# mspaintenjoyer/DepthEstimation

Hardware: AMD Instinct MI355X
Metric: disparity Mpix/s at 1080p d_max=128; 1/2/4/8-GPU scaling + %HBM roofline (higher is better)
Workload: dtype u8

## Files before the change

### depthestimation_amd/csrc/dsx_bm.hip

```cpp
#include "dsx_internal.h"
#include "dsx_partition.h"
#include "dsx_subpix.h"

constexpr int kWpe = 3;
constexpr int kWpeSsd = 4;

#ifndef DSX_ROWSTEP_PAIRTAIL
#define DSX_ROWSTEP_PAIRTAIL 0
#endif
#ifndef DSX_ROWSTEP_DIVQ
#define DSX_ROWSTEP_DIVQ 1
#endif
constexpr bool kRowstepPairtail = DSX_ROWSTEP_PAIRTAIL;
constexpr bool kRowstepDivq = DSX_ROWSTEP_DIVQ;
#ifndef DSX_ROWSTEP_ATID
#define DSX_ROWSTEP_ATID 1
#endif
#ifndef DSX_ROWSTEP_KEY2
#define DSX_ROWSTEP_KEY2 1
#endif
#ifndef DSX_ROWSTEP_MERGE
#define DSX_ROWSTEP_MERGE 1
#endif
constexpr bool kRowstepMerge = DSX_ROWSTEP_MERGE;
constexpr bool kRowstepAtid = DSX_ROWSTEP_ATID;
constexpr bool kRowstepKey2 = DSX_ROWSTEP_KEY2;

#include <algorithm>
#include <cstdio>
#include <cstdlib>
#include <cstring>
#include <mutex>
#include <type_traits>
#include <utility>
#include <vector>

namespace dsx {

typedef unsigned short u16x2 __attribute__((ext_vector_type(2)));
typedef uint32_t u32x2 __attribute__((ext_vector_type(2)));
__device__ __forceinline__ u32x2 lds_read_b64(const uint8_t *p) {
    return *(const volatile __attribute__((address_space(3))) u32x2 *)p;
}

__device__ __forceinline__ u16x2 as2(uint32_t v) { return __builtin_bit_cast(u16x2, v); }
__device__ __forceinline__ uint32_t as1(u16x2 v) { return __builtin_bit_cast(uint32_t, v); }
__device__ __forceinline__ int clampi2(int v, int lo, int hi) { return v < lo ? lo : (v > hi ? hi : v); }
__device__ __forceinline__ uint32_t umin2(uint32_t a, uint32_t b) { return a < b ? a : b; }
__device__ __forceinline__ u16x2 add_sub2(u16x2 a, u16x2 p, u16x2 q) { return as2(as1(a) + as1(p) - as1(q)); }
__device__ __forceinline__ int mad_i24(int a, int b, int c) {
    int r;
    asm("v_mad_i32_i24 %0, %1, %2, %3" : "=v"(r) : "v"(a), "v"(b), "v"(c));
    return r;
}
__device__ __forceinline__ uint32_t sad_hi_u8(uint32_t a, uint32_t b, uint32_t c) {
    return __builtin_amdgcn_sad_hi_u8(a, b, c);
}
__device__ __forceinline__ uint32_t min_shr1(uint32_t src, uint32_t key) {
    asm("s_nop 1\n\tv_min_u32_dpp %0, %1, %0 wave_shr:1 row_mask:0xf bank_mask:0xf" : "+v"(key) : "v"(src));
    return key;
}
#pragma clang diagnostic push
#pragma clang diagnostic ignored "-Winline-asm"
template <int OFF0, int STRIDE>
__device__ __forceinline__ void lds_store8_addtid(uint32_t m0base, const uint32_t (&v)[8]) {
    static_assert(OFF0 >= 0 && OFF0 + 7 * STRIDE < 65536, "16-bit offset field");
    asm volatile("s_mov_b32 m0, %8\n\ts_nop 0\n\t"
                 "ds_write_addtid_b32 %0 offset:%9\n\t"
                 "ds_write_addtid_b32 %1 offset:%10\n\t"
                 "ds_write_addtid_b32 %2 offset:%11\n\t"
                 "ds_write_addtid_b32 %3 offset:%12\n\t"
                 "ds_write_addtid_b32 %4 offset:%13\n\t"
                 "ds_write_addtid_b32 %5 offset:%14\n\t"
                 "ds_write_addtid_b32 %6 offset:%15\n\t"
                 "ds_write_addtid_b32 %7 offset:%16"
                 :
                 : "v"(v[0]), "v"(v[1]), "v"(v[2]), "v"(v[3]), "v"(v[4]), "v"(v[5]), "v"(v[6]), "v"(v[7]), "s"(m0base),
                   "n"(OFF0), "n"(OFF0 + STRIDE), "n"(OFF0 + 2 * STRIDE), "n"(OFF0 + 3 * STRIDE), "n"(OFF0 + 4 * STRIDE),
                   "n"(OFF0 + 5 * STRIDE), "n"(OFF0 + 6 * STRIDE), "n"(OFF0 + 7 * STRIDE)
                 : "memory", "m0");
}
#pragma clang diagnostic pop
__device__ __forceinline__ void lds_drain() { asm volatile("s_waitcnt lgkmcnt(0)" ::: "memory"); }
__device__ __forceinline__ uint32_t lds_offset(const uint8_t *p) {
    return (uint32_t)(uintptr_t)(const __attribute__((address_space(3))) uint8_t *)p;
}
__host__ __device__ constexpr int rnd16(int v) { return (v + 15) & ~15; }
template <int R, bool SSD, int NW>
struct Geo {
    static constexpr int TX = 32;
    static constexpr int NC = TX + 2 * R;
    static constexpr int KD = SSD ? 1 : 2;
    static constexpr int LDW = 64 * KD;
    static constexpr int Dp = NW * LDW;
    static constexpr int NT = 64 * NW;
    static constexpr int TPP = NT / TX;
    static constexpr int DSL = Dp / TPP;
    static constexpr int CB = SSD ? 4 : 2;
    static constexpr int PITCH = Dp * CB + 16;
    static constexpr int NJ = NC + Dp;
    static constexpr int REFW = rnd16(NC + 4);
    static constexpr int SROW = rnd16(NJ * 4 + 16);
    static constexpr int MAXJ = (NJ + NT - 1) / NT;
    static constexpr int NB = DSL / 8;
    static constexpr int REFB = rnd16(4 * (NC + 8));
    static constexpr int SLOT = SROW + REFB;
    static constexpr int SMEM0 = 4 * SLOT + TX * PITCH;
    static constexpr int SMEM = SMEM0 > (2 * R + 1) * SLOT ? SMEM0 : (2 * R + 1) * SLOT;
    static constexpr int XRB = 128;
};

#ifdef DSX_STAMPS
#define DSX_STAMP(i)                                                                        \
    do {                                                                                    \
        __builtin_amdgcn_sched_barrier(0);                                                  \
        uint64_t t_;                                                                        \
        asm volatile("s_memtime %0\n\ts_waitcnt lgkmcnt(0)" : "=s"(t_)::"memory");          \
        __builtin_amdgcn_sched_barrier(0);                                                  \
        if ((i) > 0) ph[(i)-1] += t_ - t_prev;                                              \
        t_prev = t_;                                                                        \
    } while (0)
#else
#define DSX_STAMP(i) \
    do {             \
    } while (0)
#endif

__device__ __forceinline__ void lds_barrier() {
    __builtin_amdgcn_fence(__ATOMIC_RELEASE, "workgroup", "local");
    __builtin_amdgcn_s_barrier();
    __builtin_amdgcn_fence(__ATOMIC_ACQUIRE, "workgroup", "local");
}

template <int NW>
__device__ __forceinline__ void block_sync() {
    if constexpr (NW == 1) {
        __builtin_amdgcn_fence(__ATOMIC_ACQ_REL, "wavefront", "local");
    } else {
        lds_barrier();
    }
}

template <int TPP>
__device__ __forceinline__ uint32_t gmin(uint32_t v) {
    if constexpr (TPP > 1) v = umin2(v, (uint32_t)__builtin_amdgcn_update_dpp(0, (int)v, 0xB1, 0xF, 0xF, false));
    if constexpr (TPP > 2) v = umin2(v, (uint32_t)__builtin_amdgcn_update_dpp(0, (int)v, 0x4E, 0xF, 0xF, false));
    if constexpr (TPP > 4) v = umin2(v, (uint32_t)__builtin_amdgcn_ds_swizzle((int)v, 0x101F));
    if constexpr (TPP > 8) v = umin2(v, (uint32_t)__builtin_amdgcn_ds_swizzle((int)v, 0x201F));
    return v;
}


typedef const __attribute__((address_space(4))) uint32_t cu32;
typedef const __attribute__((address_space(1))) uint8_t gu8;
typedef const __attribute__((address_space(1))) uint32_t gu32;
typedef __attribute__((address_space(1))) uint8_t gw8;
typedef __attribute__((address_space(1))) int16_t g16;
typedef __attribute__((address_space(1))) float gf32;

template <bool RELOAD>
__device__ __forceinline__ Bm2Args kargs_row(const Bm2Args &a) {
    if constexpr (RELOAD) {
        typedef __attribute__((address_space(4))) const Bm2Args KArgs;
        KArgs *p = (KArgs *)__builtin_amdgcn_kernarg_segment_ptr();
        asm volatile("" : "+s"(p));
// ... 231 lines not shown
            } else {
                uint32_t v = 0;
#pragma unroll
                for (int q = 0; q < 4; ++q) v |= (uint32_t)srow[clampi2(PB - 4 * tj - q, 0, W - 1)] << (8 * (3 - q));
                w = v;
                e = srow[clampi2(PB - 4 * tj - 4, 0, W - 1)];
                v = 0;
#pragma unroll
                for (int q = 0; q < 4; ++q) v |= (uint32_t)rrow[clampi2(x0 - R + 4 * tr + q, 0, W - 1)] << (8 * q);
                rf = v;
            }
        };
#pragma unroll 1
        for (int g = 0; g < NGR; ++g) {
            uint32_t w[4], e[4], rf[4];
#pragma unroll
            for (int r = 0; r < 4; ++r) {
                if (4 * g + r <= 2 * R) {
                    ldb(yb - R + 4 * g + r, w[r], e[r], rf[r]);
                } else {
                    w[r] = 0;
                    e[r] = 0;
                    rf[r] = 0;
                }
            }
            uint32_t P[5];
#pragma unroll
            for (int q = 0; q < 4; ++q) {
                const uint32_t b = 3 - q;
                const uint32_t lo = __builtin_amdgcn_perm(w[1], w[0], 0x0C0C0000u | ((4u + b) << 8) | b);
                const uint32_t hi = __builtin_amdgcn_perm(w[3], w[2], 0x0C0C0000u | ((4u + b) << 8) | b);
                P[q] = __builtin_amdgcn_perm(hi, lo, 0x05040100u);
            }
            {
                const uint32_t lo = __builtin_amdgcn_perm(e[1], e[0], 0x0C0C0400u);
                const uint32_t hi = __builtin_amdgcn_perm(e[3], e[2], 0x0C0C0400u);
                P[4] = __builtin_amdgcn_perm(hi, lo, 0x05040100u);
            }
            if (tid < NJ4) {
                uint4 *tp = reinterpret_cast<uint4 *>(smem + g * TPG + 32 * tid);
                tp[0] = make_uint4(P[0], P[1], P[1], P[2]);
                tp[1] = make_uint4(P[2], P[3], P[3], P[4]);
            }
            if (tid < NC4) {
                uint32_t Rv[4];
#pragma unroll
                for (int k = 0; k < 4; ++k) {
                    const uint32_t lo = __builtin_amdgcn_perm(rf[1], rf[0], 0x0C0C0000u | ((4u + k) << 8) | (uint32_t)k);
                    const uint32_t hi = __builtin_amdgcn_perm(rf[3], rf[2], 0x0C0C0000u | ((4u + k) << 8) | (uint32_t)k);
                    Rv[k] = __builtin_amdgcn_perm(hi, lo, 0x05040100u);
                }
                *reinterpret_cast<uint4 *>(smem + NGR * TPG + g * RG + 16 * tid) = make_uint4(Rv[0], Rv[1], Rv[2], Rv[3]);
            }
        }
        block_sync<NW>();
        const uint8_t *tb = smem + d0 * 8;
        {
        uint32_t ae[NC], ao[NC];
#pragma unroll
        for (int c = 0; c < NC; ++c) ae[c] = ao[c] = 0;
#pragma unroll 1
        for (int g = 0; g < NGR; ++g) {
#pragma unroll
            for (int q = 0; q < NC4; ++q) {
                const int c0 = 4 * q;
                const uint4 rr = *reinterpret_cast<const uint4 *>(smem + NGR * TPG + g * RG + 4 * c0);
                const uint32_t rv[4] = {rr.x, rr.y, rr.z, rr.w};
#pragma unroll
                for (int c = 0; c < 4; ++c) {
                    if (c0 + c < NC) {
                        if constexpr (ABS) {
                            const uint32_t p0 = *reinterpret_cast<const uint32_t *>(tb + g * TPG + (NC - 1 - c0 - c) * 8);
                            ae[c0 + c] = __builtin_amdgcn_sad_u8(rv[c], p0, ae[c0 + c]);
                        } else {
                            const uint2 pr = *reinterpret_cast<const uint2 *>(tb + g * TPG + (NC - 1 - c0 - c) * 8);
                            ae[c0 + c] = __builtin_amdgcn_sad_u8(rv[c], pr.x, ae[c0 + c]);
                            ao[c0 + c] = __builtin_amdgcn_sad_u8(rv[c], pr.y, ao[c0 + c]);
                        }
                    }
                }
            }
        }
#pragma unroll
        for (int c = 0; c < NC; ++c) {
            if constexpr (ABS) cs[c] = ae[c];
            else cs[c] = as2(ae[c] | (ao[c] << 16));
        }
        }

    } else {
    block_sync<NW>();
    {
        constexpr int IG = 3;
#pragma unroll 1
        for (int i0 = 0; i0 <= 2 * R; i0 += IG) {
            uint32_t iw[IG][5];
#pragma unroll
            for (int i = 0; i < IG; ++i)
                if (i0 + i <= 2 * R) ld(yb - R + i0 + i, iw[i][0], iw[i][1], iw[i][2], iw[i][3], iw[i][4]);
#pragma unroll
            for (int i = 0; i < IG; ++i)
                if (i0 + i <= 2 * R) st(i0 + i, iw[i][0], iw[i][1], iw[i][2], iw[i][3], iw[i][4]);
        }
    }
    block_sync<NW>();
#pragma unroll 1
    for (int i = 0; i <= 2 * R; ++i) {
        uint32_t nx = 0;
#pragma unroll
        for (int q = 0; q < NCH; ++q) {
            const int c0 = CW * q;
            uint32_t sw[CW + 1], rw[CW];
            float rf8[8];
            s_chunk(i, c0, sw, nx);
            if constexpr (FSS) ref_chunkf(i, c0, rf8);
            else ref_chunk(i, c0, rw);
#pragma unroll
            for (int c = 0; c < CW; ++c) {
                if (c0 + c < NC) {
                    if constexpr (FSS) {
                        const float t = rf8[c] - __uint_as_float(sw[c]);
                        cs[c0 + c] = __builtin_fmaf(t, t, cs[c0 + c]);
                    } else if constexpr (ABS) {
                        cs[c0 + c] = __builtin_amdgcn_sad_u16(rw[c], sw[c], cs[c0 + c]);
                    } else if constexpr (SSD) {
                        const int t = (int)rw[c] - (int)sw[c];
                        cs[c0 + c] += (uint32_t)__mul24(t, t);
                    } else {
                        cs[c0 + c] = as2(sad_hi_u8(rw[c], pair_e1(sw, c), __builtin_amdgcn_sad_u8(rw[c], pair_e0(sw, c), as1(cs[c0 + c]))));
                    }
                }
            }
            if constexpr (SSD) __builtin_amdgcn_sched_barrier(0);
        }
    }
    }
    block_sync<NW>();

    for (int q = tid; q < TX * (Dp - D); q += NT) {
        const int k = q / (Dp - D), d = D + (q - k * (Dp - D));
        if constexpr (SSD) *reinterpret_cast<uint32_t *>(tile + k * PITCH + d * 4) = padv + OFF;
        else *reinterpret_cast<uint16_t *>(tile + k * PITCH + d * 2) = (uint16_t)padv;
    }
    block_sync<NW>();

    const bool edge = side == 1 && (x0 + m < 0 || x0 + TX - 1 + m + Dp - 1 > W - 1);
    const bool dodd = !SSD && (D & 1);
    const bool lane_writes = d0 < D;

    uint32_t stg = (MRG ? m_lane : (uint32_t)(16 * tid)) + (uint32_t)((2 - (yb & 1) * 2) * SLOT);
    constexpr bool PTAIL = kRowstepPairtail && !SSD && SIDE == 0 && NW == 1;
    constexpr bool DIVQ = kRowstepDivq && !SSD && SIDE == 0;
    uint32_t kp0 = 0, kp1 = 0;
    for (int y = yb; y < ye; ++y) {
        const Bm2Args &a = kargs_row<SIDE == 3>(a_in);
#ifdef DSX_STAMPS
        ++nsteps;
#endif
        DSX_STAMP(0);
        if (a.prio) {
            const int dn = done0 + (y - yb);
            const int q = RL2 ? (int)(((uint32_t)(pe[0] - 1 - dn) >> 31) + ((uint32_t)(pe[1] - 1 - dn) >> 31) +
                                      ((uint32_t)(pe[2] - 1 - dn) >> 31))
                              : (dn >= pe[0]) + (dn >= pe[1]) + (dn >= pe[2]);
            if (q != qcur) {
                qcur = q;
                switch (q) {
                    case 0: __builtin_amdgcn_s_setprio(3); break;
                    case 1: __builtin_amdgcn_s_setprio(2); break;
                    case 2: __builtin_amdgcn_s_setprio(1); break;
                    default: __builtin_amdgcn_s_setprio(0); break;
                }
            }
        }
        if constexpr (RL2 && FAST && !MRG) asm volatile("" : "+v"(ofs_r), "+v"(ofs_s));
        const int par = (y & 1) * 2;
        const bool more = y + 1 < ye;
        uint32_t pn0 = 0, pn1 = 0, pn2 = 0, pn3 = 0, pnr = 0, po0 = 0, po1 = 0, po2 = 0, po3 = 0, por = 0;
        if constexpr (MRG) {
            ldm(y + 1 + R, pn0);
            ldm(y - R, po0);
        } else if (RL2 || more) {
            ld(y + 1 + R, pn0, pn1, pn2, pn3, pnr);
            ld(y - R, po0, po1, po2, po3, por);
        }
        if constexpr (FSS) {
          if (y > yb) {
#pragma unroll
            for (int q = 0; q < (NC + 3) / 4; ++q) {
                const int c0 = 4 * q;
                const uint4 rn = *reinterpret_cast<const uint4 *>(smem + par * SLOT + G::SROW + 4 * c0);
                const uint4 ro = *reinterpret_cast<const uint4 *>(smem + (par + 1) * SLOT + G::SROW + 4 * c0);
                const float rn4[4] = {__uint_as_float(rn.x), __uint_as_float(rn.y), __uint_as_float(rn.z), __uint_as_float(rn.w)};
                const float ro4[4] = {__uint_as_float(ro.x), __uint_as_float(ro.y), __uint_as_float(ro.z), __uint_as_float(ro.w)};
                const uint8_t *bn = smem + par * SLOT + d0 * 4, *bo = smem + (par + 1) * SLOT + d0 * 4;
#pragma unroll
                for (int c = 0; c < 4; ++c) {
                    if (c0 + c < NC) {
                        const float sn = *reinterpret_cast<const float *>(bn + (NC - 1 - c0 - c) * 4);
                        const float so = *reinterpret_cast<const float *>(bo + (NC - 1 - c0 - c) * 4);
                        const float tn = rn4[c] - sn, to = ro4[c] - so;
                        cs[c0 + c] = __builtin_fmaf(-to, to, __builtin_fmaf(tn, tn, cs[c0 + c]));
                    }
                }
            }
          }
        } else if (y > yb) {
            uint32_t nxn = 0, nxo = 0;
#pragma unroll
            for (int q = 0; q < NCH; ++q) {
                const int c0 = CW * q;
                uint32_t sn[CW + 1], so[CW + 1], rn[CW], ro[CW];
                ref_chunk(par, c0, rn);
                ref_chunk(par + 1, c0, ro);
                s_chunk(par, c0, sn, nxn);
                s_chunk(par + 1, c0, so, nxo);
#pragma unroll
                for (int c = 0; c < CW; ++c) {
                    if (c0 + c < NC) {
                        if constexpr (ABS) {
                            cs[c0 + c] = __builtin_amdgcn_sad_u16(rn[c], sn[c], cs[c0 + c]) -
                                         __builtin_amdgcn_sad_u16(ro[c], so[c], 0u);
                        } else if constexpr (SSD) {
                            const int tn = (int)rn[c] - (int)sn[c];
                            const int to = (int)ro[c] - (int)so[c];
                            const int nto = (int)so[c] - (int)ro[c];
                            cs[c0 + c] = (uint32_t)mad_i24(to, nto, mad_i24(tn, tn, (int)cs[c0 + c]));
                        } else {
                            const uint32_t en = sad_hi_u8(rn[c], pair_e1(sn, c), __builtin_amdgcn_sad_u8(rn[c], pair_e0(sn, c), as1(cs[c0 + c])));
                            const uint32_t lo = sad_hi_u8(ro[c], pair_e1(so, c), __builtin_amdgcn_sad_u8(ro[c], pair_e0(so, c), 0u));
                            cs[c0 + c] = as2(en - lo);
                        }
                    }
                }
            }
        }
        DSX_STAMP(1);
        DSX_STAMP(2);
        {
            uint8_t *tb = tile + d0 * CB;
            constexpr bool ATID = kRowstepAtid && !SSD && SIDE != 3;
            auto abits = [](acc_t v) __attribute__((always_inline)) -> uint32_t {
                if constexpr (FSS) return __float_as_uint(v);
                else if constexpr (SSD) return v;
                else return as1(v);
            };
            acc_t acc = cs[0];
            if constexpr (FSS) acc = 8388608.0f + cs[0];
#pragma unroll
            for (int c = 1; c <= 2 * R; ++c) {
                if constexpr (SSD) acc += cs[c];
                else acc = as2(as1(acc) + as1(cs[c]));
            }
            if constexpr (side == 3) {
                static_assert(SSD || NW <= 4, "SAD exit slots: 16 B of padding per tile row");
                const int ks = a.kshift;
                const uint32_t selE = d0 < D ? 0x05040100u : 0x0D0D0D0Du;
                const uint32_t selO = d0 + 1 < D ? 0x07060100u : 0x0D0D0D0Du;
                const uint32_t dmE = d0 < D ? (uint32_t)d0 : 0xFFFFFFFFu;
                const bool lane0 = ln == 0;
                const bool top = ln == 63;
                constexpr bool XREG = !SSD;
                uint8_t *xq = XREG ? smem + G::SMEM + G::XRB * wv : tile + Dp * CB + 4 * wv;
                constexpr int XST = XREG ? 4 : PITCH;
                uint32_t X[4] = {0xFFFFFFFFu, 0xFFFFFFFFu, 0xFFFFFFFFu, 0xFFFFFFFFu};
                uint32_t Ae = 0xFFFFFFFFu, Ao = 0xFFFFFFFFu, E = 0xFFFFFFFFu;
                auto diag_loop = [&](auto fullc) __attribute__((always_inline)) {
                    constexpr bool FULL = decltype(fullc)::value;
#pragma unroll
                    for (int k = 0; k < TX; ++k) {
                        if (k > 0) {
                            if constexpr (FSS) acc = (acc - cs[k - 1]) + cs[k + 2 * R];
                            else if constexpr (SSD) acc = acc + cs[k + 2 * R] - cs[k - 1];
                            else acc = add_sub2(acc, cs[k + 2 * R], cs[k - 1]);
                        }
                        if (FULL || lane_writes) {
                            if constexpr (SSD) *reinterpret_cast<uint32_t *>(tb + k * PITCH) = abits(acc);
                            else *reinterpret_cast<uint32_t *>(tb + k * PITCH) = as1(acc);
                        }
                        if constexpr (SSD) {
                            if (FULL || x0 + k < W) Ae = umin2(Ae, (abits(acc) << ks) | dmE);
                            if (k < TX - 1) {
                                const uint32_t F = (uint32_t)__builtin_amdgcn_mov_dpp((int)Ae, 0x13C, 0xF, 0xF, false);
                                E = (uint32_t)__builtin_amdgcn_update_dpp((int)F, (int)E, 0x138, 0xF, 0xF, false);
                                Ae = lane0 ? 0xFFFFFFFFu : F;
                            }
                        } else {
                            const uint32_t kE = __builtin_amdgcn_perm(as1(acc), (uint32_t)d0, selE);
                            const uint32_t kO = __builtin_amdgcn_perm(as1(acc), (uint32_t)(d0 + 1), selO);
                            if constexpr (FULL) {
                                if (k > 0) {
                                    const uint32_t nE = min_shr1(Ao, kE);
                                    Ao = umin2(Ae, kO);
                                    Ae = nE;
                                } else {
                                    Ae = kE;
                                    Ao = kO;
                                }
                            } else {
                                if (k > 0) {
                                    const uint32_t sh = (uint32_t)__builtin_amdgcn_update_dpp(-1, (int)Ao, 0x138, 0xF, 0xF, false);
                                    Ao = Ae;
                                    Ae = sh;
                                }
                                if (x0 + k < W) {
                                    Ae = umin2(Ae, kE);
                                    Ao = umin2(Ao, kO);
                                }
                            }
                            if (k < TX - 1) {
                                if constexpr (FULL) {
                                    X[k & 3] = Ao;
                                    if (((k & 3) == 3 || k == TX - 2) && top)
                                        *reinterpret_cast<uint4 *>(xq + (k & ~3) * 4) = make_uint4(X[0], X[1], X[2], X[3]);
                                } else if (top) {
                                    *reinterpret_cast<uint32_t *>(xq + k * XST) = Ao;
                                }
                            }
                        }
                    }
                };
                if constexpr (LRFULL) diag_loop(std::true_type{});
                else diag_loop(std::false_type{});
                uint32_t *krow = a.lr_keys + fout + (long)y * W;
                const int dtop = (wv + 1) * G::LDW - 1;
                if constexpr (SSD) {
                    const int xe = x0 + (TX - 2 - ln) - m - dtop;
                    if (ln < TX - 1 && E != 0xFFFFFFFFu && xe >= 0 && xe < W) atomicMin(krow + xe, E);
                } else if (ln < TX - 1) {
                    E = *reinterpret_cast<const uint32_t *>(xq + ln * XST);
                    const int xe = x0 + ln - m - dtop;
                    if (E != 0xFFFFFFFFu && xe >= 0 && xe < W) atomicMin(krow + xe, E);
                }
                const int xa = x0 + TX - 1 - m - d0;
                if (Ae != 0xFFFFFFFFu && xa >= 0 && xa < W) atomicMin(krow + xa, Ae);
                if constexpr (!SSD) {
                    if (Ao != 0xFFFFFFFFu && xa - 1 >= 0 && xa - 1 < W) atomicMin(krow + xa - 1, Ao);
                }
            } else if (ATID && lane_writes) {
                static_assert(!ATID || (TX % 8 == 0 && G::LDW * CB == 256), "addtid: a lane's tile bytes are 4 * lane");
                if constexpr (ATID) {
                const uint32_t mb = lds_offset(tile) + (uint32_t)wvu * (uint32_t)(G::LDW * CB);
                auto grp = [&](auto k0c) __attribute__((always_inline)) {
                    constexpr int k0 = decltype(k0c)::value;
                    uint32_t v[8];
#pragma unroll
                    for (int j = 0; j < 8; ++j) {
                        if (k0 + j > 0) acc = add_sub2(acc, cs[k0 + j + 2 * R], cs[k0 + j - 1]);
                        v[j] = as1(acc);
                    }
                    lds_store8_addtid<k0 * PITCH, PITCH>(mb, v);
                };
                grp(std::integral_constant<int, 0>{});
                grp(std::integral_constant<int, 8>{});
                grp(std::integral_constant<int, 16>{});
                grp(std::integral_constant<int, 24>{});
                }
            } else if (lane_writes) {
#pragma unroll
                for (int k = 0; k < TX; ++k) {
                    if (k > 0) {
                        if constexpr (FSS) acc = (acc - cs[k - 1]) + cs[k + 2 * R];
                        else if constexpr (SSD) acc = acc + cs[k + 2 * R] - cs[k - 1];
                        else acc = add_sub2(acc, cs[k + 2 * R], cs[k - 1]);
                    }
                    if constexpr (SSD) *reinterpret_cast<uint32_t *>(tb + k * PITCH) = abits(acc);
                    else *reinterpret_cast<uint32_t *>(tb + k * PITCH) = as1(acc);
                }
            }
            if (dodd && d0 + 1 == D) {
                for (int k = 0; k < TX; ++k) *reinterpret_cast<uint16_t *>(tb + k * PITCH + 2) = (uint16_t)padv;
            }
            if (edge && lane_writes) {
                const int base = x0 + m + d0;
                for (int k = 0; k < TX; ++k) {
                    const int p0 = base + k;
                    if constexpr (SSD) {
                        if (p0 < 0 || p0 > W - 1) *reinterpret_cast<uint32_t *>(tb + k * PITCH) = padv;
                    } else {
                        if (p0 < 0 || p0 > W - 1) *reinterpret_cast<uint16_t *>(tb + k * PITCH) = (uint16_t)padv;
                        if (p0 + 1 < 0 || p0 + 1 > W - 1) *reinterpret_cast<uint16_t *>(tb + k * PITCH + 2) = (uint16_t)padv;
                    }
                }
            }
        }
        DSX_STAMP(3);
        if constexpr (kRowstepAtid && !SSD && SIDE != 3 && NW > 1) lds_drain();
        block_sync<NW>();
        DSX_STAMP(4);
        if constexpr (RL2) {
            if constexpr (MRG) {
                if (more) {
                    stm(smem + stg, pn0);
                    stm(smem + stg + SLOT, po0);
                }
                stg = (2 * m_lane + (uint32_t)(2 * SLOT)) - stg;
            } else if constexpr (SIDE != 3) {
                if (more) {
                    st_at(smem + stg, pn0, pn1, pn2, pn3, pnr);
                    st_at(smem + stg + SLOT, po0, po1, po2, po3, por);
                }
                stg = (uint32_t)(32 * tid + 2 * SLOT) - stg;
            } else if (more) {
                st(par ^ 2, pn0, pn1, pn2, pn3, pnr);
                st((par ^ 2) + 1, po0, po1, po2, po3, por);
            }
        }
        DSX_STAMP(5);
        if constexpr (side == 2) {
            constexpr int CPP = Dp * CB / 16;
            for (int q = tid; q < TX * CPP; q += NT) {
                const int k = q / CPP, off = (q - k * CPP) * 16;
                const int x = x0 + k;
                if (x < W) {
                    const uint4 v = *reinterpret_cast<const uint4 *>(tile + k * PITCH + off);
                    *reinterpret_cast<uint4 *>(reinterpret_cast<uint8_t *>(a.vol) + ((size_t)fout + (size_t)y * W + x) * (Dp * CB) + off) = v;
                }
            }
        } else {
            const int k = tid / TPP, h = tid % TPP;
            const int x = x0 + k;
            const uint8_t *px = tile + k * PITCH + h * DSL * CB;
            uint32_t bs[NB];
#pragma unroll
            for (int i = 0; i < NB; ++i) {
                if constexpr (SSD) {
                    const uint4 v0 = *reinterpret_cast<const uint4 *>(px + 32 * i);
                    const uint4 v1 = *reinterpret_cast<const uint4 *>(px + 32 * i + 16);
                    bs[i] = umin2(umin2(umin2(v0.x, v0.y), umin2(v0.z, v0.w)), umin2(umin2(v1.x, v1.y), umin2(v1.z, v1.w))) - OFF;
                } else {
                    const uint4 v = *reinterpret_cast<const uint4 *>(px + 16 * i);
                    const u16x2 mm = __builtin_elementwise_min(__builtin_elementwise_min(as2(v.x), as2(v.y)),
                                                               __builtin_elementwise_min(as2(v.z), as2(v.w)));
                    bs[i] = umin2(mm.x, mm.y);
                }
            }
            constexpr bool KEYS = SIDE == 3 || R >= 6;
            constexpr bool KEY2 = kRowstepKey2 && !KEYS && !SSD;
            uint32_t cb, dl;
            if constexpr (KEYS) {
                constexpr int GB = Dp / 8 <= 16 ? 4 : (Dp / 8 <= 32 ? 5 : 6);
                uint32_t kmin = 0xFFFFFFFFu;
    #pragma unroll
                for (int i = 0; i < NB; ++i) kmin = umin2(kmin, (bs[i] << GB) | (uint32_t)(h * NB + i));
                kmin = gmin<TPP>(kmin);
                cb = kmin >> GB;
                const int gblk = (int)(kmin & ((1u << GB) - 1u));
                dl = 0xFFFFu;
                if (gblk / NB == h) {
                    const int bsel = gblk - h * NB;
                    uint32_t k8 = 0xFFFFFFFFu;
                    if constexpr (SSD) {
                        const uint4 v0 = *reinterpret_cast<const uint4 *>(px + 32 * bsel);
                        const uint4 v1 = *reinterpret_cast<const uint4 *>(px + 32 * bsel + 16);
                        const uint32_t c8[8] = {v0.x - OFF, v0.y - OFF, v0.z - OFF, v0.w - OFF,
                                                v1.x - OFF, v1.y - OFF, v1.z - OFF, v1.w - OFF};
    #pragma unroll
                        for (int q = 0; q < 8; ++q) k8 = umin2(k8, (c8[q] << 3) | (uint32_t)q);
                    } else {
                        const uint4 v = *reinterpret_cast<const uint4 *>(px + 16 * bsel);
                        const uint32_t w4[4] = {v.x, v.y, v.z, v.w};
    #pragma unroll
                        for (int q = 0; q < 4; ++q) {
                            k8 = umin2(k8, ((w4[q] & 0xFFFFu) << 3) | (uint32_t)(2 * q));
                            k8 = umin2(k8, ((w4[q] >> 16) << 3) | (uint32_t)(2 * q + 1));
                        }
                    }
                    dl = (uint32_t)(h * DSL + 8 * bsel + (int)(k8 & 7u));
                }
            } else if constexpr (KEY2) {
                static_assert((NB & (NB - 1)) == 0, "block index bits");
                constexpr int GB = Dp / 8 <= 16 ? 4 : (Dp / 8 <= 32 ? 5 : 6);
                uint32_t kmin = 0xFFFFFFFFu;
    #pragma unroll
                for (int i = 0; i < NB; ++i) kmin = umin2(kmin, (bs[i] << GB) | (uint32_t)i);
                kmin = gmin<TPP>(kmin | (uint32_t)(h * NB));
                cb = kmin >> GB;
                const uint32_t gblk = kmin & ((1u << GB) - 1u);
                const uint4 v = *reinterpret_cast<const uint4 *>(px + 16 * (gblk & (NB - 1)));
                const uint32_t w4[4] = {v.x, v.y, v.z, v.w};
                uint32_t k8 = 0xFFFFFFFFu;
    #pragma unroll
                for (int q = 0; q < 4; ++q) {
                    k8 = umin2(k8, (w4[q] << 16) | (uint32_t)(2 * q));
                    k8 = umin2(k8, (w4[q] & 0xFFFF0000u) | (uint32_t)(2 * q + 1));
                }
                dl = (int)(gblk / NB) == h ? gblk * 8 + (k8 & 7u) : 0xFFFFu;
            } else {
                uint32_t lmin = bs[0];
    #pragma unroll
                for (int i = 1; i < NB; ++i) lmin = umin2(lmin, bs[i]);
                cb = gmin<TPP>(lmin);
                int bsel = -1;
    #pragma unroll
                for (int i = NB - 1; i >= 0; --i) bsel = bs[i] == cb ? i : bsel;
                dl = 0xFFFFu;
                if (bsel >= 0) {
                    uint32_t c8[8];
                    if constexpr (SSD) {
                        const uint4 v0 = *reinterpret_cast<const uint4 *>(px + 32 * bsel);
                        const uint4 v1 = *reinterpret_cast<const uint4 *>(px + 32 * bsel + 16);
                        c8[0] = v0.x - OFF; c8[1] = v0.y - OFF; c8[2] = v0.z - OFF; c8[3] = v0.w - OFF;
                        c8[4] = v1.x - OFF; c8[5] = v1.y - OFF; c8[6] = v1.z - OFF; c8[7] = v1.w - OFF;
                    } else {
                        const uint4 v = *reinterpret_cast<const uint4 *>(px + 16 * bsel);
                        c8[0] = v.x & 0xFFFFu; c8[1] = v.x >> 16; c8[2] = v.y & 0xFFFFu; c8[3] = v.y >> 16;
                        c8[4] = v.z & 0xFFFFu; c8[5] = v.z >> 16; c8[6] = v.w & 0xFFFFu; c8[7] = v.w >> 16;
                    }
                    int e = 7;
    #pragma unroll
                    for (int q = 6; q >= 0; --q) e = c8[q] == cb ? q : e;
                    dl = (uint32_t)(h * DSL + 8 * bsel + e);
                }
            }
            const int b = (int)gmin<TPP>(dl);
            const long o = fout + (long)y * W + x;
            if constexpr (side == 1) {
                if (h == 0 && x < W) a.out_dR[o] = cb == padv ? (int16_t)-1 : (int16_t)b;
            } else {
                bool valid = SGK ? (x < W && x >= max(m + D, 0) && x < W + min(m, 0))
                                       : (x < W && x >= m + D - 1 && x <= W - 1 + m);
                if (a.uniq > 0) {
                    const int rel = b - h * DSL;
                    uint32_t nm = 0xFFFFFFFFu;
#pragma unroll
                    for (int i = 0; i < NB; ++i) {
                        const bool hit = rel >= 8 * i - 1 && rel <= 8 * i + 8;
                        nm = hit ? nm : umin2(nm, bs[i]);
                    }
                    const int ib0 = (rel - 1) >> 3, ib1 = (rel + 1) >> 3;
#pragma unroll
                    for (int t = 0; t < 2; ++t) {
                        const int ib = t == 0 ? ib0 : ib1;
                        if (ib >= 0 && ib < NB && (t == 0 || ib1 != ib0)) {
                            uint32_t c8[8];
                            if constexpr (SSD) {
                                const uint4 v0 = *reinterpret_cast<const uint4 *>(px + 32 * ib);
                                const uint4 v1 = *reinterpret_cast<const uint4 *>(px + 32 * ib + 16);
                                c8[0] = v0.x - OFF; c8[1] = v0.y - OFF; c8[2] = v0.z - OFF; c8[3] = v0.w - OFF;
                                c8[4] = v1.x - OFF; c8[5] = v1.y - OFF; c8[6] = v1.z - OFF; c8[7] = v1.w - OFF;
                            } else {
                                const uint4 v = *reinterpret_cast<const uint4 *>(px + 16 * ib);
                                c8[0] = v.x & 0xFFFFu; c8[1] = v.x >> 16; c8[2] = v.y & 0xFFFFu; c8[3] = v.y >> 16;
                                c8[4] = v.z & 0xFFFFu; c8[5] = v.z >> 16; c8[6] = v.w & 0xFFFFu; c8[7] = v.w >> 16;
                            }
#pragma unroll
                            for (int e = 0; e < 8; ++e) {
                                const int dd = 8 * ib + e - rel;
                                nm = (dd > 1 || dd < -1) ? umin2(nm, c8[e]) : nm;
                            }
                        }
                    }
                    nm = gmin<TPP>(nm);
                    const uint32_t real_max = padv < (1u << 24) ? padv : (1u << 24);
                    if (nm < real_max && nm * (uint32_t)(100 - a.uniq) < cb * 100u) valid = false;
                }
                if constexpr (PTAIL) {
                    const uint16_t *pc = reinterpret_cast<const uint16_t *>(tile + k * PITCH) + b;
                    u16x2 mp;
                    mp.x = pc[-1];
                    mp.y = pc[1];
                    const uint32_t c0 = (cb << 16) | ((uint32_t)valid << 15) | (uint32_t)b, c1 = as1(mp);
                    int sec = (y - yb) & 1;
                    asm("" : "+s"(sec));
                    const bool second = sec != 0;
                    if (second || !more) {
                        const bool prev = second && h == 0;
                        const uint32_t s0 = prev ? kp0 : c0, s1 = prev ? kp1 : c1;
                        const int tb = (int)(s0 & 0x7FFFu);
                        const int32_t tcb = (int32_t)(s0 >> 16), cm = (int32_t)(s1 & 0xFFFFu), cp = (int32_t)(s1 >> 16);
                        const bool tvalid = (s0 & 0x8000u) != 0;
                        int32_t f = tb * 16;
                        float pf = (float)(m + tb);
                        if (a.subpix) {
                            const bool sp = tb > 0 && tb < D - 1;
                            int32_t den = cm + cp - 2 * tcb;
                            den = den < 1 ? 1 : den;
                            const int32_t num = (cm - cp) * 16 + den;
                            const int32_t q = DIVQ ? subpix_quot(num, 2 * den) : div_trunc_small(num, 2 * den);
                            f += sp ? q : 0;
                            if (a.float_mode == 1 && sp) pf = (float)(m + tb) + (float)(cm - cp) / (float)(2 * den);
                        }
                        if ((second || h == 0) && x < W) {
                            long ro = fout + (long)(y - sec) * W;
                            asm("" : "+s"(ro));
                            const uint32_t xh = (uint32_t)(x + (h ? W : 0));
                            const int16_t fx = tvalid ? (int16_t)(m * 16 + f) : (int16_t)((m - 1) * 16);
                            if (a.out_fixed) {
                                int16_t *rowp = a.out_fixed + ro;
                                asm("" : "+s"(rowp));
                                *(g16 *)((gw8 *)rowp + 2u * xh) = fx;
                            }
                            if (a.out_float) {
                                float *rowp = a.out_float + ro;
                                asm("" : "+s"(rowp));
                                *(gf32 *)((gw8 *)rowp + 4u * xh) = a.float_mode == 0 ? (float)fx * 0.0625f : (tvalid ? pf : (float)(m - 1));
                            }
                        }
                    } else {
                        kp0 = c0;
                        kp1 = c1;
                    }
                } else {
                int32_t f = b * 16;
                float pf = (float)(m + b);
                if (a.subpix && b > 0 && b < D - 1) {
                    int32_t cm, cp;
                    const uint8_t *pk = tile + k * PITCH;
                    if constexpr (SSD) {
                        cm = (int32_t)(reinterpret_cast<const uint32_t *>(pk)[b - 1] - OFF);
                        cp = (int32_t)(reinterpret_cast<const uint32_t *>(pk)[b + 1] - OFF);
                    } else {
                        cm = reinterpret_cast<const uint16_t *>(pk)[b - 1];
                        cp = reinterpret_cast<const uint16_t *>(pk)[b + 1];
                    }
                    int32_t den = cm + cp - 2 * (int32_t)cb;
                    den = den < 1 ? 1 : den;
                    if constexpr (DIVQ) f += subpix_quot((cm - cp) * 16 + den, 2 * den);
                    else f += div_trunc_small((cm - cp) * 16 + den, 2 * den);
                    if (a.float_mode == 1) pf = (float)(m + b) + (float)(cm - cp) / (float)(2 * den);
                }
                if (h == 0 && x < W) {
                    if (lr_on) a.dstar[o] = valid ? (int16_t)b : (int16_t)-1;
                    const int16_t fx = valid ? (int16_t)(m * 16 + f) : (int16_t)((m - 1) * 16);
                    if constexpr (SGK) {
                        a.dstar[o] = fx;
                        if (valid)
                            atomicMin(a.sg_keys + fout + (long)y * W + (x - m - b),
                                      (cb << a.kshift) | (((1u << a.kshift) - 1u) - (uint32_t)b));
                    }
                    if (a.out_fixed) a.out_fixed[o] = fx;
                    if (a.out_float) a.out_float[o] = a.float_mode == 0 ? (float)fx * 0.0625f : (valid ? pf : (float)(m - 1));
                }
                }
            }
        }
        if (!RL2 && more) {
            st(par ^ 2, pn0, pn1, pn2, pn3, pnr);
            st((par ^ 2) + 1, po0, po1, po2, po3, por);
        }
        DSX_STAMP(6);
        block_sync<NW>();
        DSX_STAMP(7);
    }
}

template <int R, bool SSD, int NW, int SIDE, bool ABS>
__global__ __launch_bounds__(64 * NW) __attribute__((amdgpu_waves_per_eu((SSD && NW >= 4) ? kWpeSsd : kWpe))) void bm2(Bm2Args a) {
    using G = Geo<R, SSD, NW>;
    constexpr int TX = G::TX, NT = G::NT, NC = G::NC, NJ = G::NJ;
    constexpr int side = SIDE;
    extern __shared__ __attribute__((aligned(16))) uint8_t smem[];
    const int tid = threadIdx.x;
    const int wvu = __builtin_amdgcn_readfirstlane(tid >> 6);
    const int H = a.H, W = a.W, m = a.m;
    if (a.timeline && wvu == 0 && __lane_id() == 0) a.timeline[4 * blockIdx.x] = __builtin_amdgcn_s_memrealtime();
#ifdef DSX_STAMPS
    uint64_t ph[8] = {0, 0, 0, 0, 0, 0, 0, 0};
    uint64_t t_prev = 0;
    uint64_t nsteps = 0;
#endif

    if ((side == 0 || side == 3 || side == 4) && (a.out_fixed || a.out_float)) {
        const int xa = a.strip_begin * TX, xb = min(W, (a.strip_begin + a.strip_count) * TX);
        const int nin = xa + (W - xb);
        const int total = nin * H * a.nframes;
        const int16_t fi = (int16_t)((m - 1) * 16);
        for (int q = blockIdx.x * NT + tid; q < total; q += gridDim.x * NT) {
            const int y = q / nin;
            const int c = q - y * nin;
            const int x = c < xa ? c : xb + (c - xa);
            const long o = (long)y * W + x;
            if (a.out_fixed) a.out_fixed[o] = fi;
            if (a.out_float) a.out_float[o] = (float)(m - 1);
            if constexpr (side == 4) a.dstar[o] = fi;
        }
    }

    if ((side == 3 || side == 4) && a.lr_reset_n > 0) {
        uint32_t *kr = a.lr_reset;
        const int64_t n = a.lr_reset_n, stride = (int64_t)gridDim.x * NT;
        const int64_t t0 = (int64_t)blockIdx.x * NT + tid;
        if (((uintptr_t)kr & 15u) == 0) {
            for (int64_t q = t0; q < n / 4; q += stride)
                reinterpret_cast<uint4 *>(kr)[q] = make_uint4(0xFFFFFFFFu, 0xFFFFFFFFu, 0xFFFFFFFFu, 0xFFFFFFFFu);
            for (int64_t q = n / 4 * 4 + t0; q < n; q += stride) kr[q] = 0xFFFFFFFFu;
        } else {
            for (int64_t q = t0; q < n; q += stride) kr[q] = 0xFFFFFFFFu;
        }
    }

    const int lin0 = a.part[blockIdx.x], lin1 = a.part[blockIdx.x + 1];
    constexpr bool lr_on = SIDE == 3;
    int qcur = -1;
    int pe[3];
    {
        const int tot = lin1 - lin0;
        pe[0] = (a.pt1 * tot + 255) >> 8;
        pe[1] = (a.pt2 * tot + 255) >> 8;
        pe[2] = (a.pt3 * tot + 255) >> 8;
    }
    for (int it = lin0; it < lin1;) {
        const int sidx = it / H;
        const int f = sidx / a.strip_count;
        const int s = a.strip_begin + (sidx - f * a.strip_count);
        const long fin = (long)f * a.frame_stride, fout = (long)f * H * W;
        const int yb = it - sidx * H;
        const int ye = min(H, yb + (lin1 - it));
        const int done0 = it - lin0;
        it += ye - yb;
        const int x0 = s * TX;
        const int PB = side == 1 ? (x0 - R + m) : (x0 - R - m + NC - 1);
        const int NJ4 = (NJ + 3) / 4;
        const bool fast = (side == 1 ? (PB >= 0 && PB + 4 * NJ4 <= W - 1) : (PB - 4 * NJ4 >= 0 && PB <= W - 1)) &&
                          x0 - R >= 0 && x0 - R + 4 * ((NC + 3) / 4) - 1 <= W - 1;
#ifdef DSX_STAMPS
#define DSX_SEG(FASTV, FULLV) \
    bm2_segment<R, SSD, NW, SIDE, FASTV, ABS, FULLV>(a, smem, x0, yb, ye, fin, fout, lr_on, done0, pe, qcur, wvu, ph, t_prev, nsteps)
#else
#define DSX_SEG(FASTV, FULLV) bm2_segment<R, SSD, NW, SIDE, FASTV, ABS, FULLV>(a, smem, x0, yb, ye, fin, fout, lr_on, done0, pe, qcur, wvu)
#endif
        const bool lrfull = side == 3 && x0 + TX <= W && a.D == G::Dp;
        if (fast) {
            if (lrfull) DSX_SEG(true, true);
            else DSX_SEG(true, false);
        } else {
            if (lrfull) DSX_SEG(false, true);
            else DSX_SEG(false, false);
        }
#undef DSX_SEG
    }
    if (a.timeline && wvu == 0 && __lane_id() == 0) {
        const uint64_t t_end = __builtin_amdgcn_s_memrealtime();
        uint64_t *tl = a.timeline + 4 * blockIdx.x;
        tl[1] = t_end;
        tl[2] = (uint64_t)__builtin_amdgcn_s_getreg((4 << 0) | (0 << 6) | (31 << 11));
        tl[3] = (uint64_t)__builtin_amdgcn_s_getreg((20 << 0) | (0 << 6) | (15 << 11));
#ifdef DSX_STAMPS
        uint64_t *ps = a.timeline + 4 * 65536 + 8 * blockIdx.x;
        for (int i = 0; i < 7; ++i) ps[i] = ph[i];
        ps[7] = nsteps;
#endif
    }
}


struct PartKey {
    int dev, NG, S, sb, nframes, H, XL, XU, w8, nlev, w[4];
    bool operator==(const PartKey &o) const { return memcmp(this, &o, sizeof(PartKey)) == 0; }
};
static std::mutex &launch_mutex() {
    static std::mutex mu;
    return mu;
}
static hipError_t bm2_partition_dev(const PartKey &k, int TX, const int **out) {
    static std::vector<std::pair<PartKey, int *>> cache;
    for (const auto &e : cache)
        if (e.first == k) {
            *out = e.second;
            return hipSuccess;
        }
    if (cache.size() >= 256) {
        int prev = 0;
        (void)hipGetDevice(&prev);
        for (size_t i = 0; i < cache.size(); ++i) {
            bool seen = false;
            for (size_t j = 0; j < i; ++j) seen = seen || cache[j].first.dev == cache[i].first.dev;
            if (seen) continue;
            (void)hipSetDevice(cache[i].first.dev);
            hipError_t se = hipDeviceSynchronize();
            if (se != hipSuccess) {
                (void)hipSetDevice(prev);
                return se;
            }
        }
        for (auto &e : cache) {
            (void)hipSetDevice(e.first.dev);
            (void)hipFree(e.second);
        }
        (void)hipSetDevice(prev);
        cache.clear();
    }
    const std::vector<int> part = bm2_partition(k.NG, k.S, k.sb, k.nframes, k.H, k.XL, k.XU, TX, k.w8, k.nlev, k.w);
    int *d = nullptr;
    hipError_t e = hipMalloc(&d, part.size() * sizeof(int));
    if (e != hipSuccess) return e;
    e = hipMemcpy(d, part.data(), part.size() * sizeof(int), hipMemcpyHostToDevice);
    if (e != hipSuccess) {
        (void)hipFree(d);
        return e;
    }
    cache.emplace_back(k, d);
    *out = d;
    return hipSuccess;
}

template <int R, bool SSD, int NW, int SIDE, bool ABS = false>
// ... 135 lines not shown
```

Measured before the change: 43120.

## Overlap previous row's WTA epilogue with column SAD update and prefetch chunks

Result: faster. 44760, median of 6 (+3.8%).

```diff
diff --git a/depthestimation_amd/csrc/dsx_bm.hip b/depthestimation_amd/csrc/dsx_bm.hip
--- a/depthestimation_amd/csrc/dsx_bm.hip
+++ b/depthestimation_amd/csrc/dsx_bm.hip
@@ -11,6 +11,14 @@
 #ifndef DSX_ROWSTEP_DIVQ
 #define DSX_ROWSTEP_DIVQ 1
 #endif
+#ifndef DSX_ROWSTEP_OVERLAP
+#define DSX_ROWSTEP_OVERLAP 1
+#endif
+#ifndef DSX_ROWSTEP_AHEAD
+#define DSX_ROWSTEP_AHEAD 1
+#endif
+constexpr bool kRowstepOverlap = DSX_ROWSTEP_OVERLAP;
+constexpr bool kRowstepAhead = DSX_ROWSTEP_AHEAD;
 constexpr bool kRowstepPairtail = DSX_ROWSTEP_PAIRTAIL;
 constexpr bool kRowstepDivq = DSX_ROWSTEP_DIVQ;
 #ifndef DSX_ROWSTEP_ATID
@@ -548,6 +556,104 @@
     constexpr bool PTAIL = kRowstepPairtail && !SSD && SIDE == 0 && NW == 1;
     constexpr bool DIVQ = kRowstepDivq && !SSD && SIDE == 0;
     uint32_t kp0 = 0, kp1 = 0;
+    constexpr bool CUQ = !SSD && SIDE == 0 && NW == 1 && R < 6 && kRowstepKey2 && !PTAIL;
+    constexpr bool OVL = kRowstepOverlap && CUQ, AHD = kRowstepAhead && CUQ;
+    constexpr int CQ = 4, NQ = (NC + CQ - 1) / CQ;
+    constexpr int RPS = NQ >= 10 ? 1 : 2, NRS = 8 / RPS;
+    static_assert(NQ >= NRS + 2, "a column chunk per stage up to the element keys");
+    const int ek = tid / TPP, eh = tid % TPP, ex = x0 + ek;
+    const uint8_t *epx = tile + ek * PITCH + eh * DSL * CB;
+    uint4 etv[2] = {};
+    uint32_t ekmin = 0, ecb = 0, egblk = 0, ecm = 0, ecp = 0;
+    int eb = 0, ef = 0, eden = 1;
+    bool esp = false;
+    auto emin8 = [](uint4 v) __attribute__((always_inline)) -> uint32_t {
+        const u16x2 mm = __builtin_elementwise_min(__builtin_elementwise_min(as2(v.x), as2(v.y)),
+                                                   __builtin_elementwise_min(as2(v.z), as2(v.w)));
+        return umin2(mm.x, mm.y);
+    };
+    auto estage = [&](auto sc, int ey) __attribute__((always_inline)) {
+        constexpr int s = decltype(sc)::value;
+        static_assert(!OVL || (NB == 8 && TPP == 2), "overlapped epilogue: 64 disparities per lane, two lanes per pixel");
+        constexpr int GB = Dp / 8 <= 16 ? 4 : (Dp / 8 <= 32 ? 5 : 6);
+        if constexpr (s <= NRS) {
+            if constexpr (s == 0) ekmin = 0xFFFFFFFFu;
+#pragma unroll
+            for (int j = 0; j < (s > 0 ? RPS : 0); ++j) ekmin = umin2(ekmin, (emin8(etv[j]) << GB) | (uint32_t)(RPS * (s - 1) + j));
+            if constexpr (s < NRS) {
+#pragma unroll
+                for (int j = 0; j < RPS; ++j) etv[j] = *reinterpret_cast<const uint4 *>(epx + 16 * (RPS * s + j));
+            } else {
+                const uint32_t kmin = gmin<TPP>(ekmin | (uint32_t)(eh * 8));
+                ecb = kmin >> GB;
+                egblk = kmin & ((1u << GB) - 1u);
+                etv[0] = *reinterpret_cast<const uint4 *>(epx + 16 * (egblk & 7u));
+            }
+        } else if constexpr (s == NRS + 1) {
+            const uint32_t w4[4] = {etv[0].x, etv[0].y, etv[0].z, etv[0].w};
+            uint32_t k8 = 0xFFFFFFFFu;
+#pragma unroll
+            for (int q = 0; q < 4; ++q) {
+                k8 = umin2(k8, (w4[q] << 16) | (uint32_t)(2 * q));
+                k8 = umin2(k8, (w4[q] & 0xFFFF0000u) | (uint32_t)(2 * q + 1));
+            }
+            const uint32_t dl = (int)(egblk / 8) == eh ? egblk * 8 + (k8 & 7u) : 0xFFFFu;
+            eb = (int)gmin<TPP>(dl);
+            const uint16_t *pc = reinterpret_cast<const uint16_t *>(tile + ek * PITCH) + eb;
+            ecm = pc[-1];
+            ecp = pc[1];
+        } else if constexpr (s == NRS + 2) {
+            esp = a.subpix && eb > 0 && eb < D - 1;
+            int32_t den = (int32_t)ecm + (int32_t)ecp - 2 * (int32_t)ecb;
+            eden = den < 1 ? 1 : den;
+            const int32_t num = ((int32_t)ecm - (int32_t)ecp) * 16 + eden;
+            const int32_t q = DIVQ ? subpix_quot(num, 2 * eden) : div_trunc_small(num, 2 * eden);
+            ef = eb * 16 + (esp ? q : 0);
+        } else {
+            bool valid = ex < W && ex >= m + D - 1 && ex <= W - 1 + m;
+            if (a.uniq > 0) {
+                const int rel = eb - eh * DSL;
+                uint32_t nm = 0xFFFFFFFFu;
+#pragma unroll
+                for (int i = 0; i < 8; ++i) {
+                    const bool hit = rel >= 8 * i - 1 && rel <= 8 * i + 8;
+                    nm = hit ? nm : umin2(nm, emin8(*reinterpret_cast<const uint4 *>(epx + 16 * i)));
+                }
+                const int ib0 = (rel - 1) >> 3, ib1 = (rel + 1) >> 3;
+#pragma unroll
+                for (int t = 0; t < 2; ++t) {
+                    const int ib = t == 0 ? ib0 : ib1;
+                    if (ib >= 0 && ib < 8 && (t == 0 || ib1 != ib0)) {
+                        const uint4 v = *reinterpret_cast<const uint4 *>(epx + 16 * ib);
+                        const uint32_t c8[8] = {v.x & 0xFFFFu, v.x >> 16, v.y & 0xFFFFu, v.y >> 16,
+                                                v.z & 0xFFFFu, v.z >> 16, v.w & 0xFFFFu, v.w >> 16};
+#pragma unroll
+                        for (int e = 0; e < 8; ++e) {
+                            const int dd = 8 * ib + e - rel;
+                            nm = (dd > 1 || dd < -1) ? umin2(nm, c8[e]) : nm;
+                        }
+                    }
+                }
+                nm = gmin<TPP>(nm);
+                const uint32_t real_max = padv < (1u << 24) ? padv : (1u << 24);
+                if (nm < real_max && nm * (uint32_t)(100 - a.uniq) < ecb * 100u) valid = false;
+            }
+            if (eh == 0 && ex < W) {
+                const long o = fout + (long)ey * W + ex;
+                const int16_t fx = valid ? (int16_t)(m * 16 + ef) : (int16_t)((m - 1) * 16);
+                if (a.out_fixed) a.out_fixed[o] = fx;
+                if (a.out_float) {
+                    if (a.float_mode == 0) {
+                        a.out_float[o] = (float)fx * 0.0625f;
+                    } else {
+                        float pf = (float)(m + eb);
+                        if (esp) pf = (float)(m + eb) + (float)((int32_t)ecm - (int32_t)ecp) / (float)(2 * eden);
+                        a.out_float[o] = valid ? pf : (float)(m - 1);
+                    }
+                }
+            }
+        }
+    };
     for (int y = yb; y < ye; ++y) {
         const Bm2Args &a = kargs_row<SIDE == 3>(a_in);
 #ifdef DSX_STAMPS
@@ -599,6 +705,68 @@
                         cs[c0 + c] = __builtin_fmaf(-to, to, __builtin_fmaf(tn, tn, cs[c0 + c]));
                     }
                 }
+            }
+          }
+        } else if constexpr (OVL || AHD) {
+          if (y > yb) {
+            uint32_t sn[2][CQ + 1], so[2][CQ + 1], rn[2][CQ], ro[2][CQ];
+            uint32_t nxn = 0, nxo = 0;
+            auto rd = [&](auto qc) __attribute__((always_inline)) {
+                constexpr int q = decltype(qc)::value, c0 = CQ * q, t = AHD ? (q & 1) : 0;
+                const uint8_t *bn = (const uint8_t *)__builtin_assume_aligned(smem + par * SLOT + d0 * 4, 8);
+                const uint8_t *bo = (const uint8_t *)__builtin_assume_aligned(smem + (par + 1) * SLOT + d0 * 4, 8);
+                const uint4 vn = *reinterpret_cast<const uint4 *>(smem + par * SLOT + G::SROW + 4 * c0);
+                const uint4 vo = *reinterpret_cast<const uint4 *>(smem + (par + 1) * SLOT + G::SROW + 4 * c0);
+                rn[t][0] = vn.x; rn[t][1] = vn.y; rn[t][2] = vn.z; rn[t][3] = vn.w;
+                ro[t][0] = vo.x; ro[t][1] = vo.y; ro[t][2] = vo.z; ro[t][3] = vo.w;
+                sn[t][0] = c0 == 0 ? *reinterpret_cast<const uint32_t *>(bn + NC * 4) : nxn;
+                so[t][0] = c0 == 0 ? *reinterpret_cast<const uint32_t *>(bo + NC * 4) : nxo;
+#pragma unroll
+                for (int c = 1; c < CQ; c += 2) {
+                    if (c0 + c < NC) {
+                        const u32x2 pn = lds_read_b64(bn + (NC - 1 - c0 - c) * 4);
+                        const u32x2 po = lds_read_b64(bo + (NC - 1 - c0 - c) * 4);
+                        sn[t][c + 1] = pn.x; sn[t][c] = pn.y; nxn = pn.x;
+                        so[t][c + 1] = po.x; so[t][c] = po.y; nxo = po.x;
+                    }
+                }
+            };
+            auto sads = [&](auto qc) __attribute__((always_inline)) {
+                constexpr int q = decltype(qc)::value, c0 = CQ * q, t = AHD ? (q & 1) : 0;
+#pragma unroll
+                for (int c = 0; c < CQ; ++c) {
+                    if (c0 + c < NC) {
+                        const uint32_t en = sad_hi_u8(rn[t][c], sn[t][c], __builtin_amdgcn_sad_u8(rn[t][c], sn[t][c + 1], as1(cs[c0 + c])));
+                        const uint32_t lo = sad_hi_u8(ro[t][c], so[t][c], __builtin_amdgcn_sad_u8(ro[t][c], so[t][c + 1], 0u));
+                        uint32_t v = en - lo;
+                        if constexpr (OVL) asm volatile("" : "+v"(v));
+                        cs[c0 + c] = as2(v);
+                    }
+                }
+            };
+            auto chunk = [&](auto qc) __attribute__((always_inline)) {
+                constexpr int q = decltype(qc)::value;
+                if constexpr (q < NQ) {
+                    __builtin_amdgcn_sched_barrier(0);
+                    if constexpr (OVL && q < NRS + 3) estage(qc, y - 1);
+                    if constexpr (!AHD) rd(qc);
+                    else if constexpr (q + 1 < NQ) rd(std::integral_constant<int, q + 1>{});
+                    __builtin_amdgcn_sched_barrier(0);
+                    sads(qc);
+                }
+            };
+            if constexpr (AHD) rd(std::integral_constant<int, 0>{});
+            chunk(std::integral_constant<int, 0>{}); chunk(std::integral_constant<int, 1>{});
+            chunk(std::integral_constant<int, 2>{}); chunk(std::integral_constant<int, 3>{});
+            chunk(std::integral_constant<int, 4>{}); chunk(std::integral_constant<int, 5>{});
+            chunk(std::integral_constant<int, 6>{}); chunk(std::integral_constant<int, 7>{});
+            chunk(std::integral_constant<int, 8>{}); chunk(std::integral_constant<int, 9>{});
+            chunk(std::integral_constant<int, 10>{}); chunk(std::integral_constant<int, 11>{});
+            static_assert(NQ <= 12 && NQ >= 7, "chunks of the overlapped column update");
+            __builtin_amdgcn_sched_barrier(0);
+            if constexpr (OVL) {
+                if constexpr (NQ < NRS + 3) estage(std::integral_constant<int, NRS + 2>{}, y - 1);
+                estage(std::integral_constant<int, NRS + 3>{}, y - 1);
             }
           }
         } else if (y > yb) {
@@ -813,7 +981,7 @@
                     *reinterpret_cast<uint4 *>(reinterpret_cast<uint8_t *>(a.vol) + ((size_t)fout + (size_t)y * W + x) * (Dp * CB) + off) = v;
                 }
             }
-        } else {
+        } else if constexpr (!OVL) {
             const int k = tid / TPP, h = tid % TPP;
             const int x = x0 + k;
             const uint8_t *px = tile + k * PITCH + h * DSL * CB;
@@ -1039,6 +1207,15 @@
         block_sync<NW>();
         DSX_STAMP(7);
     }
+    if constexpr (OVL) {
+        auto dr = [&](auto sc) __attribute__((always_inline)) {
+            if constexpr (decltype(sc)::value <= NRS + 3) estage(sc, ye - 1);
+        };
+        dr(std::integral_constant<int, 0>{}); dr(std::integral_constant<int, 1>{}); dr(std::integral_constant<int, 2>{});
+        dr(std::integral_constant<int, 3>{}); dr(std::integral_constant<int, 4>{}); dr(std::integral_constant<int, 5>{});
+        dr(std::integral_constant<int, 6>{}); dr(std::integral_constant<int, 7>{}); dr(std::integral_constant<int, 8>{});
+        dr(std::integral_constant<int, 9>{}); dr(std::integral_constant<int, 10>{}); dr(std::integral_constant<int, 11>{});
+    }
 }
 
 template <int R, bool SSD, int NW, int SIDE, bool ABS>
```
